# delldu/VSTNet

Measured on AMD Instinct MI355X. Metric: stylized frames/sec at 1024x1024 (1/2/4/8 GPU) + % HBM roofline, higher is better.
Workload: dtype bf16x3

## Files before the change

include/vstnet.h:

```cpp
#ifndef VSTNET_H
#define VSTNET_H

#include <stddef.h>
#include <stdint.h>

#ifdef __cplusplus
extern "C" {
#endif
#pragma GCC visibility push(default)

#define VST_OK 0
#define VST_E_ARG (-1)
#define VST_E_SHAPE (-2)
#define VST_E_MODE (-3)
#define VST_E_WORKSPACE (-4)

#define VST_PREC_BF16X3 0
#define VST_PREC_FP32 1
#define VST_PREC_F16X2 2

#define VST_PREC_F16X2H 3

#define VST_NUM_BLOCKS 32

// ... 160 lines not shown
int vst_cwct_factor_n_f64(const double* content_stats, const double* const* style_stats_host_array, const float* alphas_host,
                          int n_styles, float alpha_c, float eps, int N, double* affine, int* info, void* workspace,
                          size_t workspace_bytes, void* stream);
int vst_cwct_apply_n_f64(const float* x, float* y, int N, long L, const double* affine, const uint8_t* mask, int label,
                         void* stream);

#define VST_KERNEL_ID(cin, cout, stride) (((cin) << 16) | ((cout) << 4) | (stride))
#define VST_KERNEL_ALL (-1)
#define VST_KERNEL_PACK 1
#define VST_KERNEL_UNPACK 2
#define VST_KERNEL_SPREAD 3
#define VST_KERNEL_GATHER 4
#define VST_KERNEL_CWCT_STATS 5
#define VST_KERNEL_CWCT_FACTOR 6
#define VST_KERNEL_CWCT_APPLY 7
#define VST_KERNEL_PRESPLIT 8
int vst_profile_begin(int kernel_id, int max_records);
int vst_profile_end(double* total_ms, int* launches);
int vst_profile_end_table(int* ids, double* ms, int* launches, int cap, int* n_ids);

#define VST_OPT_STAGE3_LEAN 1
#define VST_OPT_STAGE3_PINGPONG 2
#define VST_OPT_STAGE3_WIDE 3
int vst_set_option(int option, int value);
int vst_get_option(int option);

#pragma GCC visibility pop
#ifdef __cplusplus
}
#endif
#endif
```

vstnet_amd/_lib.py:

```python
from __future__ import annotations

import ctypes as C
import glob
import os
import subprocess

PKG_DIR = os.path.dirname(os.path.abspath(__file__))
REPO_DIR = os.path.dirname(PKG_DIR)
LIB_PATH = os.environ.get("VSTNET_HIP_LIB") or os.path.join(PKG_DIR, "libvstnet_hip.so")
RESOURCES_PATH = os.path.join(PKG_DIR, "libvstnet_hip.resources.txt")
SOURCES = sorted(glob.glob(os.path.join(PKG_DIR, "csrc", "*.hip")))
HEADERS = sorted(glob.glob(os.path.join(PKG_DIR, "csrc", "*.h"))) + [os.path.join(REPO_DIR, "include", "vstnet.h")]

NUM_BLOCKS = 32
PREC_BF16X3 = 0
PREC_FP32 = 1
PREC_F16X2 = 2
PREC_F16X2H = 3

EXPORTS = [
    "vst_version", "vst_error_string", "vst_conv_packed_bytes", "vst_pack_conv", "vst_pack_input",
    "vst_unpack_output", "vst_pack_input_u8", "vst_unpack_output_u8", "vst_revnet_forward_u8", "vst_revnet_inverse_u8",
    "vst_spread", "vst_gather", "vst_block_tmp_bytes", "vst_block_apply",
    "vst_pass_workspace_bytes", "vst_revnet_forward", "vst_revnet_inverse",
# ... 4 lines not shown
    "vst_cwct_stats_code_workspace_bytes", "vst_cwct_stats_code", "vst_cwct_apply_code",
    "vst_mask_to_code", "vst_cwct_stats_labels_code_workspace_bytes", "vst_cwct_stats_labels_code", "vst_cwct_apply_labels_code",
    "vst_revnet_decode_labels", "vst_revnet_decode_labels_u8", "vst_pass_sub_batch",
    "vst_normalize_block", "vst_range_flags", "vst_range_flags_async",
    "vst_cwct_stats_f64_workspace_bytes", "vst_cwct_stats_f64", "vst_cwct_factor_f64_workspace_bytes", "vst_cwct_factor_f64",
    "vst_cwct_apply_f64",
    "vst_generic_conv", "vst_generic_squeeze", "vst_generic_unsqueeze", "vst_generic_copy_channels", "vst_generic_zero",
    "vst_set_option", "vst_get_option",
    "vst_cwct_stats_n_workspace_bytes", "vst_cwct_stats_n", "vst_cwct_factor_n_workspace_bytes", "vst_cwct_factor_n",
    "vst_cwct_prefactor_n", "vst_cwct_apply_n", "vst_cwct_stats_n_f64_workspace_bytes", "vst_cwct_stats_n_f64",
    "vst_cwct_factor_n_f64_workspace_bytes", "vst_cwct_factor_n_f64", "vst_cwct_apply_n_f64",
    "vst_max_frame_pixels", "vst_cwct_stats_code_rect", "vst_cwct_stats_labels_code_rect",
    "vst_colors_to_labels", "vst_label_hist", "vst_mask_prepare", "vst_remap_lut", "vst_apply_lut", "vst_label_plan_hist",
    "vst_cwct_factor_labels_keyed",
    "vst_label_plan_hists", "vst_cwct_factor_labels_mix", "vst_cwct_prefactor_labels",
]
MAX_STYLES = 8
MASK_OVERFLOW = 1
MASK_OUT_OF_TABLE = 2
LABEL_PLAN_BYTES = 2344
OPT_STAGE3_LEAN = 1
OPT_STAGE3_PINGPONG = 2
OPT_STAGE3_WIDE = 3
RANGE_SATURATED = 1
RANGE_WEIGHT = 2


PRECISIONS = {"bf16x3": PREC_BF16X3, "fp32": PREC_FP32, "f16x2": PREC_F16X2, "f16x2h": PREC_F16X2H}


def default_precision() -> str:
    p = os.environ.get("VST_PRECISION", "bf16x3")
    if p not in PRECISIONS:
        raise ValueError(f"VST_PRECISION must be one of {sorted(PRECISIONS)}")
    return p


class VstError(RuntimeError):
    pass


class ConvWeights(C.Structure):
    _fields_ = [("packed", C.c_void_p), ("bias", C.c_void_p)]


class BlockWeights(C.Structure):
# ... 205 lines not shown
```

vstnet_amd/csrc/conv.hip:

```cpp
#include <mutex>
#include <stdlib.h>
#include "common.h"

#ifndef VST_ABLATE
#define VST_ABLATE 0
#endif

struct ConvArgs {
    const float* in;
    float* out;
    const unsigned char* packed;
    const float* bias;
    int Hin, Win, Hout, Wout;
    int Wq;
    size_t in_img_stride;
    size_t out_img_stride;
    float sign;
    int tiles_x, tiles_y, tiles_total;
    const unsigned char* packed1;
    const float* bias1;
    unsigned char* out_sp;
    size_t out_sp_img_bytes;
    unsigned trace_base;
};

#ifndef VST_XCD_REMAP
#define VST_XCD_REMAP 1
#endif
#ifndef VST_PIPE_OLD_SPREAD
#define VST_PIPE_OLD_SPREAD 1
#endif
#ifndef VST_PIPE_NO_DEFER
#define VST_PIPE_NO_DEFER 0
#endif
#ifdef VST_TRACE
__device__ unsigned long long vst_trace_buf[4 * 16384];
__device__ unsigned long long* vst_trace_ptr;
__device__ unsigned vst_trace_cap;
static std::atomic<unsigned> vst_trace_host_n{0};
#define VST_TRACE_RESERVE(t_, grid_) (t_).trace_base = vst_trace_host_n.fetch_add((unsigned)(grid_));
#define VST_TRACE_BEGIN(which)                                                                                  \
    const unsigned long long trace_t0 = __builtin_amdgcn_s_memrealtime();
#define VST_TRACE_END_(which, cin_, cout_)                                                                      \
    if (VST_TRACE == (which) || VST_TRACE == 3) {                                                               \
        __builtin_amdgcn_s_waitcnt(0);                                                                          \
        asm volatile("s_waitcnt vmcnt(0)" ::: "memory");                                                       \
// ... 29 lines not shown
    (void)zero;
    vst_trace_host_n.store(0);
    return (int)e;
}
extern "C" __attribute__((visibility("default"))) int vst_trace_count(unsigned* n) { *n = vst_trace_host_n.load(); return 0; }
#else
#define VST_TRACE_BEGIN(which)
#define VST_TRACE_END(which)
#define VST_TRACE_END_(which, cin_, cout_)
#define VST_TRACE_RESERVE(t_, grid_)
#endif

__device__ __forceinline__ bool xcd_tile(const ConvArgs& a, int& bx, int& by, int& bz) {
    const int g = blockIdx.x, per = gridDim.x >> 3;
    const int n = VST_XCD_REMAP ? (g & 7) * per + (g >> 3) : g;
    if (n >= a.tiles_total) return false;
    bx = n % a.tiles_x;
    const int r = n / a.tiles_x;
    by = r % a.tiles_y;
    bz = r / a.tiles_y;
    return true;
}

template <int CIN, int COUT, int STRIDE, int MRO = 0>
struct ConvCfg {
    static constexpr int NT = COUT >= 64 ? 64 : 16;
    static constexpr int NB = NT / 16;
    static constexpr int COUTP = (COUT + 15) / 16 * 16;
    static constexpr int NCOT = COUTP / NT;
    static constexpr int MR = MRO ? MRO : (STRIDE == 2 ? 2 : 4);
    static constexpr int TH = 4 * MR, TW = 16;
    static constexpr int IH = (TH - 1) * STRIDE + 3, IW = (TW - 1) * STRIDE + 3;
    static constexpr int NSLOT = (IH * IW + 15) / 16 * 16;
    static constexpr int CC = CIN >= 32 ? 32 : CIN;
    static constexpr int NCHUNK = CIN / CC;
    static constexpr int CIG = CC >= 8 ? CC / 8 : 1;
#ifndef VST_ABLATE_KS16
#define VST_ABLATE_KS16 5
#endif
    static constexpr int KS = CIN >= 32 ? 9 : (CIN == 16 ? VST_ABLATE_KS16 : 2);
    static constexpr int A_PLANE = CIN == 4 ? NSLOT * 8 : CIG * NSLOT * 16;
    static constexpr int B_PLANE = KS * 4 * NT * 16;
    static constexpr int LDS_BYTES = 2 * A_PLANE + 2 * B_PLANE;
    static constexpr int LDS_BYTES_T2 = 2 * A_PLANE + B_PLANE;
    static_assert(LDS_BYTES <= 160 * 1024, "LDS budget");
};

__device__ __forceinline__ void split8_f16(const float4 v0, const float4 v1, uint4& hi, uint4& lo, float& amax) {
    const float f[8] = {v0.x, v0.y, v0.z, v0.w, v1.x, v1.y, v1.z, v1.w};
    u32x4 h, l;
    split8_sp(f, h, l, amax);
    hi = __builtin_bit_cast(uint4, h);
    lo = __builtin_bit_cast(uint4, l);
}

__device__ __forceinline__ void split4_f16(const float4 v, uint2& hi, uint2& lo, float& amax) {
    const float f[4] = {v.x, v.y, v.z, v.w};
    typedef __attribute__((ext_vector_type(4))) _Float16 f16x4;
    f16x4 h, l;
#ifndef VST_NO_RANGE_CHECK
    amax = fmaxf(fmaxf(amax, fabsf(f[0])), fmaxf(fmaxf(fabsf(f[1]), fabsf(f[2])), fabsf(f[3])));
#endif
#pragma unroll
// ... 77 lines not shown
            }
            *p = r;
        }
}

#define MFMA3(acc, wh, wl, xh, xl)                                              \
    acc = __builtin_amdgcn_mfma_f32_16x16x32_bf16(wh, xl, acc, 0, 0, 0);        \
    acc = __builtin_amdgcn_mfma_f32_16x16x32_bf16(wl, xh, acc, 0, 0, 0);        \
    acc = __builtin_amdgcn_mfma_f32_16x16x32_bf16(wh, xh, acc, 0, 0, 0)

#define MFMA_T(acc, wh, wl, xh, xl)                                                                                          \
    if constexpr (TERMS == 3) {                                                                                               \
        MFMA3(acc, wh, wl, xh, xl);                                                                                           \
    } else {                                                                                                                  \
        acc = __builtin_amdgcn_mfma_f32_16x16x32_f16(__builtin_bit_cast(f16x8, wh), __builtin_bit_cast(f16x8, xl), acc, 0, 0, 0); \
        acc = __builtin_amdgcn_mfma_f32_16x16x32_f16(__builtin_bit_cast(f16x8, wh), __builtin_bit_cast(f16x8, xh), acc, 0, 0, 0); \
    }
#define SPLIT8_T(v0_, v1_, h_, l_) { if constexpr (TERMS == 3) split8(v0_, v1_, h_, l_); else split8_f16(v0_, v1_, h_, l_, range_amax); }
#define SPLIT4_T(v_, h_, l_) { if constexpr (TERMS == 3) split4(v_, h_, l_); else split4_f16(v_, h_, l_, range_amax); }

#ifndef VST_EARLY_OLD
#define VST_EARLY_OLD 1
#endif
template <int CIN, int COUT, int STRIDE, bool IN_STATE, bool OUT_STATE, bool OUT_SP = false, int TERMS = 3, bool OUT_H16 = false>
__global__ __launch_bounds__(256) void conv_mfma_kernel(const ConvArgs a) {
    using C = ConvCfg<CIN, COUT, STRIDE>;
    extern __shared__ __attribute__((aligned(16))) unsigned char smem[];
    unsigned char* const a_hi = smem;
    unsigned char* const a_lo = smem + C::A_PLANE;
    unsigned char* const b_hi = smem + 2 * C::A_PLANE;
    unsigned char* const b_lo = TERMS == 3 ? b_hi + C::B_PLANE : b_hi;

    const int tid = threadIdx.x, lane = tid & 63, wave = tid >> 6;
    const int lrow = lane & 15, kg = lane >> 4;
    int bx, by, bz;
    if (!xcd_tile(a, bx, by, bz)) return;
    float range_amax = 0.f;
    VST_TRACE_BEGIN(2)
    const int tx0 = bx * C::TW, ty0 = by * C::TH;
    const int b = bz / C::NCOT, co0 = (bz % C::NCOT) * C::NT;

    const float* const in_img = a.in + (size_t)b * a.in_img_stride;
    const PackedConvLayout PL = packed_conv_layout(COUT, CIN);
    const unsigned char* const w_hi = a.packed + (TERMS == 3 ? PL.f32_bytes : PL.f16_offset);
    const unsigned char* const w_lo = w_hi + PL.frag_bytes;

    f32x4 acc[C::MR][C::NB];
#pragma unroll
    for (int m = 0; m < C::MR; ++m)
#pragma unroll
        for (int n = 0; n < C::NB; ++n) acc[m][n] = f32x4{0.f, 0.f, 0.f, 0.f};

    const int slot_base = (wave * C::MR * STRIDE) * C::IW + lrow * STRIDE;

    constexpr int A_ITEMS_T = CIN == 4 ? C::IH * C::IW : C::IH * C::IW * C::CIG;
    constexpr int AIT = (A_ITEMS_T + 255) / 256, NV = CIN == 4 ? 1 : 2;
    constexpr int W_ITEMS_T = C::KS * 4 * C::NT, WIT = (W_ITEMS_T + 255) / 256;
    typedef __attribute__((ext_vector_type(4))) unsigned u32x4;
    f32x4 areg[AIT][NV];
    u32x4 wreg[WIT][2];
#define F4(v_) make_float4((v_)[0], (v_)[1], (v_)[2], (v_)[3])
#define GEN_FETCH(chunk_)                                                                           \
    _Pragma("unroll") for (int it = 0; it < WIT; ++it) {                                           \
        int idx = it * 256 + tid;                                                                  \
        idx = idx < W_ITEMS_T ? idx : W_ITEMS_T - 1;                                               \
        const int co = idx % C::NT, r = idx / C::NT;                                               \
        const size_t src = ((size_t)((chunk_) * C::KS * 4 + r) * C::COUTP + co0 + co) * 16;        \
        wreg[it][0] = *(const u32x4*)(w_hi + src);                                                 \
        if (TERMS == 3) wreg[it][1] = *(const u32x4*)(w_lo + src);                                 \
    }                                                                                              \
    _Pragma("unroll") for (int it = 0; it < AIT; ++it) {                                           \
        int idx = it * 256 + tid;                                                                  \
        idx = idx < A_ITEMS_T ? idx : A_ITEMS_T - 1;                                               \
        const int cig = CIN == 4 ? 0 : idx % C::CIG, slot = CIN == 4 ? idx : idx / C::CIG;         \
        const int iy = slot / C::IW, ix = slot - iy * C::IW;                                       \
        const int gy = reflect_clamp(ty0 * STRIDE - 1 + iy, a.Hin);                                \
        const int gx = reflect_clamp(tx0 * STRIDE - 1 + ix, a.Win);                                \
        const size_t off = IN_STATE ? zc_offset(vst_level_of_channels(CIN), gy, gx, a.Wq)          \
                                    : ((size_t)gy * a.Win + gx) * CIN;                             \
        const float* p = in_img + off + (chunk_) * C::CC + cig * 8;                                \
        areg[it][0] = *(const f32x4*)p;                                                            \
        if (NV == 2) areg[it][NV - 1] = *(const f32x4*)(p + 4);                                    \
    }
#define GEN_LAND()                                                                                 \
    _Pragma("unroll") for (int it = 0; it < AIT; ++it) {                                           \
        int idx = it * 256 + tid;                                                                  \
        idx = idx < A_ITEMS_T ? idx : A_ITEMS_T - 1;                                               \
        if (CIN == 4) {                                                                            \
            uint2 h, l;                                                                            \
            SPLIT4_T(F4(areg[it][0]), h, l);                                                       \
            *(uint2*)(a_hi + idx * 8) = h;                                                         \
            *(uint2*)(a_lo + idx * 8) = l;                                                         \
// ... 3 lines not shown
            SPLIT8_T(F4(areg[it][0]), F4(areg[it][NV - 1]), h, l);                                 \
            *(uint4*)(a_hi + (cig * C::NSLOT + slot) * 16) = h;                                    \
            *(uint4*)(a_lo + (cig * C::NSLOT + slot) * 16) = l;                                    \
        }                                                                                          \
    }                                                                                              \
    _Pragma("unroll") for (int it = 0; it < WIT; ++it) {                                           \
        int idx = it * 256 + tid;                                                                  \
        idx = idx < W_ITEMS_T ? idx : W_ITEMS_T - 1;                                               \
        *(u32x4*)(b_hi + idx * 16) = wreg[it][0];                                                  \
        if (TERMS == 3) *(u32x4*)(b_lo + idx * 16) = wreg[it][1];                                  \
    }

    float* const out_img = a.out + (size_t)b * a.out_img_stride;
    float4 bias[C::NB], old[C::MR][C::NB];
    const bool interior = COUT % 16 == 0 && ty0 + C::TH <= a.Hout && tx0 + C::TW <= a.Wout;
    constexpr bool EARLY_OLD = OUT_STATE && VST_EARLY_OLD && C::MR * C::NB >= 16;
    auto fetch_old = [&]() __attribute__((always_inline)) {
        if (interior) load_old<COUT, C::MR, C::NB, true>(a, out_img, ty0 + wave * C::MR, tx0 + lrow, co0 + 4 * kg, old);
        else load_old<COUT, C::MR, C::NB>(a, out_img, ty0 + wave * C::MR, tx0 + lrow, co0 + 4 * kg, old);
    };

    GEN_FETCH(0);
    GEN_LAND();
#pragma unroll
    for (int chunk = 0; chunk < C::NCHUNK; ++chunk) {
        __syncthreads();
        if (chunk + 1 < C::NCHUNK) { GEN_FETCH(chunk + 1); }
        if (EARLY_OLD && chunk == C::NCHUNK - 1) fetch_old();

#pragma unroll
        for (int ks = 0; ks < C::KS; ++ks) {
            bf16x8 wh[C::NB], wl[C::NB];
#pragma unroll
            for (int n = 0; n < C::NB; ++n) {
                const int boff = ((ks * 4 + kg) * C::NT + n * 16 + lrow) * 16;
                wh[n] = __builtin_bit_cast(bf16x8, *(const uint4*)(b_hi + boff));
                if (TERMS == 3) wl[n] = __builtin_bit_cast(bf16x8, *(const uint4*)(b_lo + boff)); else wl[n] = wh[n];
            }
#pragma unroll
            for (int m = 0; m < C::MR; ++m) {
                bf16x8 xh, xl;
                if (CIN >= 32) {
                    const int dy = ks / 3, dx = ks - dy * 3;
                    const int slot = slot_base + (m * STRIDE + dy) * C::IW + dx;
                    const int aoff = (kg * C::NSLOT + slot) * 16;
                    xh = __builtin_bit_cast(bf16x8, *(const uint4*)(a_hi + aoff));
// ... 104 lines not shown
        xh = __builtin_bit_cast(bf16x8, make_uint4(h0.x, h0.y, h1.x, h1.y));
        if (!NO_LO) {
            const uint2 l0 = *(const uint2*)(img_lo + s0 * 8), l1 = *(const uint2*)(img_lo + s1 * 8);
            xl = __builtin_bit_cast(bf16x8, make_uint4(l0.x, l0.y, l1.x, l1.y));
        } else {
            xl = xh;
        }
    }
}

template <int MID, int CH, int TERMS = 3, int MR = 4, bool H16 = false>
struct PairCfg {
    using C7 = ConvCfg<MID, CH, 1, MR>;
    static constexpr int R1 = 20, N1SLOT = (4 * MR + 4) * R1, RW = 18, RH = 4 * MR + 2, NPX = RH * RW, NBLK = (NPX + 15) / 16;
    static constexpr int H1_PLANE = MID == 4 ? N1SLOT * 8 : C7::CIG * N1SLOT * 16;
    static constexpr int W4_PLANE = C7::KS * 4 * 16 * 16;
    static constexpr bool ALIAS = MID == 16;
    static constexpr int WPL = TERMS == 3 ? 2 : 1;
    static constexpr int H1W4 = (H16 ? 1 : 2) * H1_PLANE + WPL * W4_PLANE;
    static constexpr int U_BYTES = ALIAS ? (H1W4 > WPL * C7::B_PLANE ? H1W4 : WPL * C7::B_PLANE) : H1W4 + WPL * C7::B_PLANE;
    static constexpr int LDS_BYTES = 2 * C7::A_PLANE + U_BYTES;
};

template <int MID, int CH, int TERMS = 3, int MR = 4, bool H16 = false>
__global__ __launch_bounds__(256, (MID == 16 && TERMS == 2) ? 3 : 1) void conv_pair_kernel(const ConvArgs a) {
    static_assert(!H16 || TERMS == 2, "fp16 h1: the 2-term kernels only");
    using P = PairCfg<MID, CH, TERMS, MR, H16>;
    using C = typename P::C7;
    static_assert(C::NCHUNK == 1 && C::NCOT == 1, "single-chunk shapes");
    extern __shared__ __attribute__((aligned(16))) unsigned char smem[];
    unsigned char* const a_hi = smem;
    unsigned char* const a_lo = smem + C::A_PLANE;
    unsigned char* const u0 = smem + 2 * C::A_PLANE;
    unsigned char* const b_hi = P::ALIAS ? u0 : u0 + P::H1W4;
    unsigned char* const b_lo = TERMS == 3 ? b_hi + C::B_PLANE : b_hi;
    unsigned char* const h1_hi = u0;
    unsigned char* const h1_lo = H16 ? u0 : u0 + P::H1_PLANE;
    unsigned char* const w4s_hi = u0 + (H16 ? 1 : 2) * P::H1_PLANE;
    unsigned char* const w4s_lo = TERMS == 3 ? w4s_hi + P::W4_PLANE : w4s_hi;

    const int tid = threadIdx.x, lane = tid & 63, wave = tid >> 6;
    const int lrow = lane & 15, kg = lane >> 4;
    int bx, by, b;
    if (!xcd_tile(a, bx, by, b)) return;
    float range_amax = 0.f;
    VST_TRACE_BEGIN(1)
    const int tx0 = bx * C::TW, ty0 = by * C::TH;
    const int H = a.Hout, W = a.Wout;
    const float* const in_img = a.in + (size_t)b * a.in_img_stride;
// ... 26 lines not shown
        const int iy = slot / P::R1, ix = slot - iy * P::R1;
        const int gy = reflect_clamp(ty0 - 2 + iy, H), gx = reflect_clamp(tx0 - 2 + ix, W);
        if constexpr (H16) {
            const _Float16* p16 = (const _Float16*)a.in + (size_t)b * a.in_img_stride + ((size_t)gy * W + gx) * MID + cig * 8;
            if (MID == 4) { const uint2 v = *(const uint2*)p16; h16reg[it] = u32x4{v.x, v.y, 0u, 0u}; }
            else h16reg[it] = *(const u32x4*)p16;
        } else {
            const float* p = in_img + ((size_t)gy * W + gx) * MID + cig * 8;
            hreg[it][0] = *(const f32x4*)p;
            if (NV == 2) hreg[it][NV - 1] = *(const f32x4*)(p + 4);
        }
    }
#pragma unroll
    for (int it = 0; it < W7IT; ++it) {
        int idx = it * 256 + tid;
        idx = idx < W7_ITEMS ? idx : W7_ITEMS - 1;
        const int co = idx % C::NT, r = idx / C::NT;
        const size_t src = ((size_t)r * C::COUTP + co) * 16;
        w7reg[it][0] = *(const u32x4*)(w7_hi + src);
        if (TERMS == 3) w7reg[it][1] = *(const u32x4*)(w7_lo + src);
    }
    float4 bias[C::NB], old[C::MR][C::NB];
    const bool interior = ty0 + C::TH <= H && tx0 + C::TW <= W;
    constexpr bool EARLY_OLD = C::MR * C::NB >= 16 && TERMS == 3;
#define PAIR_FETCH_OLD()                                                                                         \
    if (interior) load_old<CH, C::MR, C::NB, true>(a, out_img, ty0 + wave * C::MR, tx0 + lrow, 4 * kg, old);   \
    else load_old<CH, C::MR, C::NB>(a, out_img, ty0 + wave * C::MR, tx0 + lrow, 4 * kg, old);
    if (EARLY_OLD) { PAIR_FETCH_OLD(); }

#define F4(v_) make_float4((v_)[0], (v_)[1], (v_)[2], (v_)[3])
#pragma unroll
    for (int it = 0; it < H1IT; ++it) {
        int idx = it * 256 + tid;
        idx = idx < H1_ITEMS ? idx : H1_ITEMS - 1;
        if constexpr (H16) {
            if (MID == 4) {
                *(uint2*)(h1_hi + idx * 8) = make_uint2(h16reg[it][0], h16reg[it][1]);
            } else {
                const int cig = idx % C::CIG, slot = idx / C::CIG;
                *(u32x4*)(h1_hi + (cig * P::N1SLOT + slot) * 16) = h16reg[it];
            }
        } else if (MID == 4) {
            uint2 h, l;
            SPLIT4_T(F4(hreg[it][0]), h, l);
            *(uint2*)(h1_hi + idx * 8) = h;
            *(uint2*)(h1_lo + idx * 8) = l;
        } else {
// ... 117 lines not shown
    for (int m = 0; m < C::MR; ++m)
#pragma unroll
        for (int n = 0; n < C::NB; ++n) acc[m][n] = f32x4{0.f, 0.f, 0.f, 0.f};
    const int slot_base = (wave * C::MR) * C::IW + lrow;
#pragma unroll
    for (int ks = 0; ks < C::KS; ++ks) {
        bf16x8 wh[C::NB], wl[C::NB];
#pragma unroll
        for (int n = 0; n < C::NB; ++n) {
            const int boff = ((ks * 4 + kg) * C::NT + n * 16 + lrow) * 16;
            wh[n] = __builtin_bit_cast(bf16x8, *(const uint4*)(b_hi + boff));
            wl[n] = __builtin_bit_cast(bf16x8, *(const uint4*)(b_lo + boff));
        }
#pragma unroll
        for (int m = 0; m < C::MR; ++m) {
            bf16x8 xh, xl;
            read_x_small<MID>(a_hi, a_lo, C::NSLOT, slot_base + m * C::IW, C::IW, ks, kg, xh, xl);
#pragma unroll
            for (int n = 0; n < C::NB; ++n) { MFMA_T(acc[m][n], wh[n], wl[n], xh, xl); }
        }
    }
    load_bias<CH, C::NB>(a, 4 * kg, bias);
    if constexpr (TERMS == 2) vst_note_range(range_amax);
    if (!EARLY_OLD) { PAIR_FETCH_OLD(); }
#undef PAIR_FETCH_OLD
    if (interior) store_tile<CH, true, C::MR, C::NB, true>(a, out_img, ty0 + wave * C::MR, tx0 + lrow, 4 * kg, acc, bias, old);
    else store_tile<CH, true, C::MR, C::NB>(a, out_img, ty0 + wave * C::MR, tx0 + lrow, 4 * kg, acc, bias, old);
    VST_TRACE_END_(1, MID, CH)
}

#ifdef VST_PP_STAMP
__device__ unsigned long long vst_pp_stamps[2 * 32 * 8];
extern "C" __attribute__((visibility("default"))) int vst_pp_stamps_dump(unsigned long long* host) {
    return (int)hipMemcpyFromSymbol(host, HIP_SYMBOL(vst_pp_stamps), sizeof(vst_pp_stamps));
}
#define PP_STAMP(grp_, st_, k_)                                                                                  \
    if (blockIdx.x == 128 && lane == 0 && (wave & 3) == 0 && (st_) < 32) {                                       \
        asm volatile("s_waitcnt lgkmcnt(0)" ::: "memory");                                                      \
        vst_pp_stamps[((grp_) * 32 + (st_)) * 8 + (k_)] = __builtin_amdgcn_s_memtime();                          \
    }
__device__ unsigned long long vst_pp_clk[4];
extern "C" __attribute__((visibility("default"))) int vst_pp_clk_dump(unsigned long long* host) {
    return (int)hipMemcpyFromSymbol(host, HIP_SYMBOL(vst_pp_clk), sizeof(vst_pp_clk));
}
#define PP_CLK(i_)                                                                                               \
    if (blockIdx.x == 128 && threadIdx.x == 0) {                                                                 \
// ... 665 lines not shown
    (void)hipEventRecord(g_prof_ev[2 * rec], st);
    return rec;
}

void vst_prof_close(int rec, hipStream_t st) {
    std::lock_guard<std::mutex> lk(g_prof_mu);
    if (rec < g_prof_count) (void)hipEventRecord(g_prof_ev[2 * rec + 1], st);
}

#ifndef VST_LEAN_DEFAULT
#define VST_LEAN_DEFAULT 0
#endif
static std::atomic<int> g_opt_lean{[] { const char* e = getenv("VST_LEAN"); return e && (e[0] == '0' || e[0] == '1') ? e[0] - '0' : VST_LEAN_DEFAULT; }()};
static bool vst_lean_stage3() { return g_opt_lean.load(std::memory_order_relaxed) != 0; }
#ifndef VST_WIDE_DEFAULT
#define VST_WIDE_DEFAULT 1
#endif
static std::atomic<int> g_opt_wide{[] { const char* e = getenv("VST_WIDE"); return e && (e[0] == '0' || e[0] == '1') ? e[0] - '0' : VST_WIDE_DEFAULT; }()};
#ifndef VST_PINGPONG_DEFAULT
#define VST_PINGPONG_DEFAULT 0
#endif
static std::atomic<int> g_opt_pp{[] { const char* e = getenv("VST_PINGPONG"); return e && (e[0] == '0' || e[0] == '1') ? e[0] - '0' : VST_PINGPONG_DEFAULT; }()};

template <int CIN, int COUT, int STRIDE, bool IN_STATE, bool OUT_STATE>
static int launch_conv(const ConvArgs& a, int B, int precision, hipStream_t st, bool out_h16 = false) {
    if (precision == VST_PREC_FP32) {
        const size_t total = (size_t)B * a.Hout * a.Wout * COUT;
        size_t blocks = (total + 255) / 256;
        if (blocks > 65536) blocks = 65536;
        conv_fp32_kernel<IN_STATE, OUT_STATE><<<dim3((unsigned)blocks), 256, 0, st>>>(a, CIN, COUT, STRIDE, B);
        VST_RETURN_IF_LAUNCH_FAILED();
        return VST_OK;
    }
    if (precision != VST_PREC_BF16X3 && !vst_is_f16(precision)) return VST_E_MODE;
    vst_prof_scope prof(VST_KERNEL_ID(CIN, COUT, STRIDE), st);
    if constexpr (CIN >= 64 && COUT >= 64 && STRIDE == 1) {
        ConvArgs t = a;
        t.tiles_x = (a.Wout + 15) / 16;
        if (vst_lean_stage3()) {
            using C = PipeCfg<CIN, COUT, 4>;
            auto kern = conv_pipe_kernel<CIN, COUT, IN_STATE, OUT_STATE, 4>;
            static std::atomic<unsigned> attr_done{0};
            if (int rc_ = vst_ensure_dynamic_lds((const void*)kern, (int)(C::LDS_BYTES), &attr_done)) return rc_;
            t.tiles_y = (a.Hout + C::TH - 1) / C::TH; t.tiles_total = t.tiles_x * t.tiles_y * B;
            VST_TRACE_RESERVE(t, (t.tiles_total + 7) / 8 * 8)
            kern<<<dim3((t.tiles_total + 7) / 8 * 8), C::NTHR, C::LDS_BYTES, st>>>(t);
// ... 14 lines not shown
            if (int rc_ = vst_ensure_dynamic_lds((const void*)kern, lds, &attr_done)) return rc_;
            t.tiles_y = (a.Hout + C::TH - 1) / C::TH; t.tiles_total = t.tiles_x * t.tiles_y * B;
            VST_TRACE_RESERVE(t, (t.tiles_total + 7) / 8 * 8)
            kern<<<dim3((t.tiles_total + 7) / 8 * 8), C::NTHR, lds, st>>>(t);
#endif
        } else {
            using C = PipeCfg<CIN, COUT>;
            auto kern = conv_pipe_kernel<CIN, COUT, IN_STATE, OUT_STATE>;
            static std::atomic<unsigned> attr_done{0};
            if (int rc_ = vst_ensure_dynamic_lds((const void*)kern, (int)(C::LDS_BYTES), &attr_done)) return rc_;
            t.tiles_y = (a.Hout + C::TH - 1) / C::TH; t.tiles_total = t.tiles_x * t.tiles_y * B;
            VST_TRACE_RESERVE(t, (t.tiles_total + 7) / 8 * 8)
            kern<<<dim3((t.tiles_total + 7) / 8 * 8), C::NTHR, C::LDS_BYTES, st>>>(t);
        }
    } else {
        using C = ConvCfg<CIN, COUT, STRIDE>;
        constexpr bool T2_SHAPE = (CIN == 64 && COUT == 16) || (CIN == 16 && COUT == 16 && STRIDE == 2) || (CIN == 16 && COUT == 4);
        const bool t2 = T2_SHAPE && vst_is_f16(precision);
        constexpr bool H16_SHAPE = T2_SHAPE && !OUT_STATE;
        const bool h16 = t2 && out_h16 && H16_SHAPE;
        auto kern = h16 ? conv_mfma_kernel<CIN, COUT, STRIDE, IN_STATE, OUT_STATE, false, T2_SHAPE ? 2 : 3, H16_SHAPE>
                  : t2 ? conv_mfma_kernel<CIN, COUT, STRIDE, IN_STATE, OUT_STATE, false, T2_SHAPE ? 2 : 3>
                       : conv_mfma_kernel<CIN, COUT, STRIDE, IN_STATE, OUT_STATE, false, 3>;
        const int lds = t2 ? C::LDS_BYTES_T2 : C::LDS_BYTES;
        static std::atomic<unsigned> attr_done[3];
        if (int rc_ = vst_ensure_dynamic_lds((const void*)kern, lds, &attr_done[h16 ? 2 : (t2 ? 1 : 0)])) return rc_;
        ConvArgs t = a;
        t.tiles_x = (a.Wout + C::TW - 1) / C::TW; t.tiles_y = (a.Hout + C::TH - 1) / C::TH;
        t.tiles_total = t.tiles_x * t.tiles_y * B * C::NCOT;
        VST_TRACE_RESERVE(t, (t.tiles_total + 7) / 8 * 8)
        kern<<<dim3((t.tiles_total + 7) / 8 * 8), 256, lds, st>>>(t);
    }
    VST_RETURN_IF_LAUNCH_FAILED();
    return VST_OK;
}

static int launch_conv_s2_planes(const ConvArgs& a, int B, hipStream_t st) {
    using C = ConvCfg<64, 64, 2>;
    vst_prof_scope prof(VST_KERNEL_ID(64, 64, 2), st);
    auto kern = conv_mfma_kernel<64, 64, 2, true, false, true, 2>;
    static std::atomic<unsigned> attr_done{0};
    if (int rc_ = vst_ensure_dynamic_lds((const void*)kern, (int)(C::LDS_BYTES_T2), &attr_done)) return rc_;
    ConvArgs t = a;
    t.tiles_x = (a.Wout + C::TW - 1) / C::TW; t.tiles_y = (a.Hout + C::TH - 1) / C::TH;
    t.tiles_total = t.tiles_x * t.tiles_y * B * C::NCOT;
    VST_TRACE_RESERVE(t, (t.tiles_total + 7) / 8 * 8)
    kern<<<dim3((t.tiles_total + 7) / 8 * 8), 256, C::LDS_BYTES_T2, st>>>(t);
    VST_RETURN_IF_LAUNCH_FAILED();
    return VST_OK;
}

#ifndef VST_PAIR
#define VST_PAIR 1
#endif
#ifndef VST_PAIR_MR2_T3
#define VST_PAIR_MR2_T3 0
#endif
#ifndef VST_PAIR_MR2
#define VST_PAIR_MR2 0
#endif
template <int MID, int CH>
static int launch_pair(const ConvArgs& a, int B, int precision, hipStream_t st) {
    constexpr int T2 = 2;
    const bool t2 = T2 == 2 && vst_is_f16(precision);
    if (precision == VST_PREC_F16X2H) {
        using P = PairCfg<MID, CH, 2, 4, true>;
        vst_prof_scope prof(VST_KERNEL_ID(MID, CH, 1), st);
        auto kern = conv_pair_kernel<MID, CH, 2, 4, true>;
        static std::atomic<unsigned> attr_h16{0};
        if (int rc_ = vst_ensure_dynamic_lds((const void*)kern, P::LDS_BYTES, &attr_h16)) return rc_;
        ConvArgs t = a;
        t.tiles_x = (a.Wout + 15) / 16; t.tiles_y = (a.Hout + 15) / 16; t.tiles_total = t.tiles_x * t.tiles_y * B;
        VST_TRACE_RESERVE(t, (t.tiles_total + 7) / 8 * 8)
        kern<<<dim3((t.tiles_total + 7) / 8 * 8), 256, P::LDS_BYTES, st>>>(t);
        VST_RETURN_IF_LAUNCH_FAILED();
        return VST_OK;
    }
    vst_prof_scope prof(VST_KERNEL_ID(MID, CH, 1), st);
    constexpr int MRT = (MID == 16 && VST_PAIR_MR2) ? 2 : 4;
    constexpr int MRT3 = (MID == 16 && VST_PAIR_MR2_T3) ? 2 : 4;
    auto kern = t2 ? conv_pair_kernel<MID, CH, T2, MRT> : conv_pair_kernel<MID, CH, 3, MRT3>;
    const int lds = t2 ? PairCfg<MID, CH, T2, MRT>::LDS_BYTES : PairCfg<MID, CH, 3, MRT3>::LDS_BYTES;
    const int th = t2 ? 4 * MRT : 4 * MRT3;
    static std::atomic<unsigned> attr_done[2];
    if (int rc_ = vst_ensure_dynamic_lds((const void*)kern, lds, &attr_done[t2 ? 1 : 0])) return rc_;
    ConvArgs t = a;
    t.tiles_x = (a.Wout + 15) / 16; t.tiles_y = (a.Hout + th - 1) / th; t.tiles_total = t.tiles_x * t.tiles_y * B;
    VST_TRACE_RESERVE(t, (t.tiles_total + 7) / 8 * 8)
    kern<<<dim3((t.tiles_total + 7) / 8 * 8), 256, lds, st>>>(t);
    VST_RETURN_IF_LAUNCH_FAILED();
    return VST_OK;
}

template <int CH, int STRIDE>
static int run_block(const vst_block_weights* w, int direction, int precision, float* dst, const float* src,
                     float* tmp, int B, int H, int W, hipStream_t st) {
    constexpr int LV = CH == 16 ? 0 : (CH == 64 ? 1 : 2);
    constexpr int MID = CH / 4;
    constexpr int IN_CH = STRIDE == 1 ? CH : CH / 4;
    const int Ho = H >> LV, Wo = W >> LV;
    const size_t state_img = (size_t)H * W * 16;
    const size_t mid_img = (size_t)Ho * Wo * MID;
    float* h1 = tmp;
    float* h2 = tmp + (size_t)B * mid_img;
    ConvArgs a{};
    a.Wq = W >> 2;
    a.in = src; a.out = h1; a.packed = (const unsigned char*)w->conv[0].packed; a.bias = w->conv[0].bias;
    a.Hin = Ho * STRIDE; a.Win = Wo * STRIDE; a.Hout = Ho; a.Wout = Wo;
    a.in_img_stride = state_img; a.out_img_stride = mid_img; a.sign = 0.f;
    if constexpr (CH == 256 && STRIDE == 2) {
        if (vst_is_f16(precision)) {
            const size_t mid_bytes = (size_t)Ho * Wo * 64 * 4, state_bytes = (size_t)Ho * Wo * 256 * 4;
            unsigned char* const h1p = (unsigned char*)tmp;
            unsigned char* const h2p = h1p + (size_t)B * mid_bytes;
            unsigned char* const planes_a = h2p + (size_t)B * mid_bytes;
            (void)state_bytes;
            a.out_sp = h1p; a.out_sp_img_bytes = mid_bytes;
            int rc2 = launch_conv_s2_planes(a, B, st);
            if (rc2) return rc2;
            const int h2_single = precision == VST_PREC_F16X2H;
            rc2 = vst3_conv_mid(&w->conv[1], h1p, h2p, h2_single, B, H, W, st);
            if (rc2) return rc2;
            return vst3_conv_out(&w->conv[2], h2p, h2_single, dst, direction > 0 ? planes_a : nullptr, direction > 0 ? 1.f : -1.f,
                                 B, H, W, st);
        }
    }
    const bool h16 = CH <= 64 && VST_PAIR && precision == VST_PREC_F16X2H;
    int rc = launch_conv<IN_CH, MID, STRIDE, true, false>(a, B, precision, st, h16);
    if (rc) return rc;
    if constexpr (CH <= 64 && VST_PAIR) {
        if (precision != VST_PREC_FP32) {
            a.in = h1; a.out = dst; a.Hin = Ho; a.Win = Wo; a.in_img_stride = mid_img; a.out_img_stride = state_img;
            a.packed = (const unsigned char*)w->conv[2].packed; a.bias = w->conv[2].bias;
            a.packed1 = (const unsigned char*)w->conv[1].packed; a.bias1 = w->conv[1].bias;
            a.sign = direction > 0 ? 1.f : -1.f;
            return launch_pair<MID, CH>(a, B, precision, st);
        }
    }
    a.in = h1; a.out = h2; a.packed = (const unsigned char*)w->conv[1].packed; a.bias = w->conv[1].bias;
    a.Hin = Ho; a.Win = Wo; a.in_img_stride = mid_img;
    rc = launch_conv<MID, MID, 1, false, false>(a, B, precision, st);
    if (rc) return rc;
    a.in = h2; a.out = dst; a.packed = (const unsigned char*)w->conv[2].packed; a.bias = w->conv[2].bias;
    a.out_img_stride = state_img; a.sign = direction > 0 ? 1.f : -1.f;
    return launch_conv<MID, CH, 1, false, true>(a, B, precision, st);
}

static const int kBlockChannel[VST_NUM_BLOCKS] = {16, 16, 16, 16, 16, 16, 16, 16, 16, 16, 64, 64, 64, 64, 64, 64,
                                                  64, 64, 64, 64, 256, 256, 256, 256, 256, 256, 256, 256, 256, 256,
                                                  256, 256};
static const int kBlockStride[VST_NUM_BLOCKS] = {1, 1, 1, 1, 1, 1, 1, 1, 1, 1, 2, 1, 1, 1, 1, 1,
                                                 1, 1, 1, 1, 2, 1, 1, 1, 1, 1, 1, 1, 1, 1, 1, 1};

VST_DEFINE_TU_RANGE(vst_range_tu_conv)

extern "C" {

int vst_set_option(int option, int value) {
    if (option == VST_OPT_STAGE3_LEAN) g_opt_lean.store(value != 0, std::memory_order_relaxed);
    else if (option == VST_OPT_STAGE3_WIDE) g_opt_wide.store(value != 0, std::memory_order_relaxed);
    else if (option == VST_OPT_STAGE3_PINGPONG && VST_WITH_PINGPONG) g_opt_pp.store(value != 0, std::memory_order_relaxed);
    else return VST_E_ARG;
    return VST_OK;
}

int vst_get_option(int option) {
    if (option == VST_OPT_STAGE3_LEAN) return g_opt_lean.load(std::memory_order_relaxed);
    if (option == VST_OPT_STAGE3_WIDE) return g_opt_wide.load(std::memory_order_relaxed);
    if (option == VST_OPT_STAGE3_PINGPONG && VST_WITH_PINGPONG) return g_opt_pp.load(std::memory_order_relaxed);
    return VST_E_ARG;
}

int vst_range_flags(unsigned* flags_host, int reset) {
    if (!flags_host) return VST_E_ARG;
    hipError_t e = hipDeviceSynchronize();
    if (e != hipSuccess) return (int)e;
    unsigned v = 0;
    if (int rc = vst_range_tu_conv(&v, reset)) return rc;
    if (int rc = vst_range_tu_conv3(&v, reset)) return rc;
    if (int rc = vst_range_tu_layout(&v, reset)) return rc;
    if (int rc = vst_range_tu_cwct(&v, reset)) return rc;
    *flags_host = v;
    return VST_OK;
}

int vst_range_flags_async(unsigned* flags4_dev, void* stream) {
    if (!flags4_dev) return VST_E_ARG;
    hipStream_t st = (hipStream_t)stream;
    if (int rc = vst_range_tu_conv_async(flags4_dev + 0, st)) return rc;
    if (int rc = vst_range_tu_conv3_async(flags4_dev + 1, st)) return rc;
    if (int rc = vst_range_tu_layout_async(flags4_dev + 2, st)) return rc;
    return vst_range_tu_cwct_async(flags4_dev + 3, st);
// ... 108 lines not shown
        else
            rc = vst_block_apply(&w->blocks[k], kBlockChannel[k], kBlockStride[k], +1, precision, s[k & 1], s[1 - (k & 1)],
                                 tmp, B, H, W, stream);
        if (rc) return rc;
    }
    return VST_OK;
}

static int revnet_forward_chunk(const vst_net_weights* w, const float* x, const uint8_t* x_u8, float* z, void* workspace,
                                int B, int C_in, int H, int W, int sp_steps, int precision, void* stream) {
    float* s[2];
    s[0] = (float*)workspace;
    s[1] = s[0] + (size_t)B * H * W * 16;
    float* tmp = s[1] + (size_t)B * H * W * 16;
    const int rc = forward_blocks(w, x, x_u8, s, tmp, B, C_in, H, W, precision, stream);
    if (rc) return rc;
    return vst_spread(s[0], s[1], z, B, H, W, sp_steps, stream);
}

static int inverse_blocks(const vst_net_weights* w, float* x, uint8_t* x_u8, float* const s[2], float* tmp, int B, int C_out,
                          int H, int W, int precision, void* stream) {
    const bool sp = vst_is_f16(precision);
    int rc = VST_OK;
    for (int k = VST_NUM_BLOCKS - 1; k >= 0; --k) {
        if (sp && k >= 21)
            rc = vst3_block256(&w->blocks[k], -1, precision, s[k & 1], s[1 - (k & 1)], tmp, VST_NUM_BLOCKS - 1 - k, 1, B, H, W,
                               stream);
        else
            rc = vst_block_apply(&w->blocks[k], kBlockChannel[k], kBlockStride[k], -1, precision, s[k & 1], s[1 - (k & 1)],
                                 tmp, B, H, W, stream);
        if (rc) return rc;
    }
    return x_u8 ? vst_unpack_output_u8(s[0], x_u8, B, H, W, stream) : vst_unpack_output(s[0], x, B, C_out, H, W, stream);
}

static int revnet_inverse_chunk(const vst_net_weights* w, const float* z, float* x, uint8_t* x_u8, void* workspace, int B,
                                int C_out, int H, int W, int sp_steps, int precision, void* stream) {
    float* s[2];
    s[0] = (float*)workspace;
    s[1] = s[0] + (size_t)B * H * W * 16;
    float* tmp = s[1] + (size_t)B * H * W * 16;
    const bool sp = vst_is_f16(precision);
    const int rc = sp ? vst3_gather_planes(z, vst3_plane_buffer(tmp, 0, B, H, W), s[1], B, H, W, sp_steps, stream)
                      : vst_gather(z, s[0], s[1], B, H, W, sp_steps, stream);
    if (rc) return rc;
    return inverse_blocks(w, x, x_u8, s, tmp, B, C_out, H, W, precision, stream);
}

static int revnet_encode_any(const vst_net_weights* w, const float* x, const uint8_t* x_u8, float* code, void* workspace, int B,
                             int C_in, int H, int W, int precision, void* stream) {
// ... 187 lines not shown
```

Before: 217.5.

## Fold 3x3 taps for 16-to-4 conv and fuse final block with RGB output

Adds a tap-folded form of the 16-channel-in, 4-channel-out conv. It treats the spatial taps as MFMA output rows and sums the shifted partial results through LDS, so the MFMA does not waste lanes padding 4 output channels to 16. It also fuses the last inverse block's pair kernel with the output unpack, writing planar float or u8 RGB directly and skipping the separate unpack pass and the state write. Both paths are on by default and controlled by new options. The cost is extra LDS transposes and syncs in the folded kernel and more special-case code paths.

```diff
diff --git a/include/vstnet.h b/include/vstnet.h
--- a/include/vstnet.h
+++ b/include/vstnet.h
@@ -206,6 +206,8 @@
 #define VST_OPT_STAGE3_LEAN 1
 #define VST_OPT_STAGE3_PINGPONG 2
 #define VST_OPT_STAGE3_WIDE 3
+#define VST_OPT_STAGE1_FOLD 4
+#define VST_OPT_OUT_RGB 5
 int vst_set_option(int option, int value);
 int vst_get_option(int option);
 
diff --git a/vstnet_amd/_lib.py b/vstnet_amd/_lib.py
--- a/vstnet_amd/_lib.py
+++ b/vstnet_amd/_lib.py
@@ -50,6 +50,8 @@
 OPT_STAGE3_LEAN = 1
 OPT_STAGE3_PINGPONG = 2
 OPT_STAGE3_WIDE = 3
+OPT_STAGE1_FOLD = 4
+OPT_OUT_RGB = 5
 RANGE_SATURATED = 1
 RANGE_WEIGHT = 2
 
diff --git a/vstnet_amd/csrc/conv.hip b/vstnet_amd/csrc/conv.hip
--- a/vstnet_amd/csrc/conv.hip
+++ b/vstnet_amd/csrc/conv.hip
@@ -22,6 +22,9 @@
     unsigned char* out_sp;
     size_t out_sp_img_bytes;
     unsigned trace_base;
+    float* rgb;
+    unsigned char* rgb_u8;
+    int rgb_c;
 };
 
 #ifndef VST_XCD_REMAP
@@ -97,7 +100,7 @@
     return true;
 }
 
-template <int CIN, int COUT, int STRIDE, int MRO = 0>
+template <int CIN, int COUT, int STRIDE, int MRO = 0, int KSO = 0>
 struct ConvCfg {
     static constexpr int NT = COUT >= 64 ? 64 : 16;
     static constexpr int NB = NT / 16;
@@ -113,7 +116,7 @@
 #ifndef VST_ABLATE_KS16
 #define VST_ABLATE_KS16 5
 #endif
-    static constexpr int KS = CIN >= 32 ? 9 : (CIN == 16 ? VST_ABLATE_KS16 : 2);
+    static constexpr int KS = KSO ? KSO : (CIN >= 32 ? 9 : (CIN == 16 ? VST_ABLATE_KS16 : 2));
     static constexpr int A_PLANE = CIN == 4 ? NSLOT * 8 : CIG * NSLOT * 16;
     static constexpr int B_PLANE = KS * 4 * NT * 16;
     static constexpr int LDS_BYTES = 2 * A_PLANE + 2 * B_PLANE;
@@ -237,9 +240,12 @@
 #ifndef VST_EARLY_OLD
 #define VST_EARLY_OLD 1
 #endif
-template <int CIN, int COUT, int STRIDE, bool IN_STATE, bool OUT_STATE, bool OUT_SP = false, int TERMS = 3, bool OUT_H16 = false>
+template <int CIN, int COUT, int STRIDE, bool IN_STATE, bool OUT_STATE, bool OUT_SP = false, int TERMS = 3, bool OUT_H16 = false,
+          bool FOLD = false>
 __global__ __launch_bounds__(256) void conv_mfma_kernel(const ConvArgs a) {
-    using C = ConvCfg<CIN, COUT, STRIDE>;
+    static_assert(!FOLD || (CIN == 16 && COUT == 4 && STRIDE == 1 && TERMS == 3 && !OUT_STATE && !OUT_SP && !OUT_H16),
+                  "tap-folded form: conv.1 of the 16-channel blocks, bf16x3");
+    using C = ConvCfg<CIN, COUT, STRIDE, 0, FOLD ? 2 : 0>;
     extern __shared__ __attribute__((aligned(16))) unsigned char smem[];
     unsigned char* const a_hi = smem;
     unsigned char* const a_lo = smem + C::A_PLANE;
@@ -280,9 +286,19 @@
         int idx = it * 256 + tid;                                                                  \
         idx = idx < W_ITEMS_T ? idx : W_ITEMS_T - 1;                                               \
         const int co = idx % C::NT, r = idx / C::NT;                                               \
-        const size_t src = ((size_t)((chunk_) * C::KS * 4 + r) * C::COUTP + co0 + co) * 16;        \
-        wreg[it][0] = *(const u32x4*)(w_hi + src);                                                 \
-        if (TERMS == 3) wreg[it][1] = *(const u32x4*)(w_lo + src);                                 \
+        if constexpr (FOLD) {                                                                      \
+            const int ty = 2 * (r >> 2) + ((r >> 1) & 1), tx = co >> 2;           \
+            const bool live = ty < 3 && tx < 3;                                                    \
+            const int tap = live ? 3 * ty + tx : 0;                                                \
+            const size_t src = ((size_t)((tap >> 1) * 4 + (tap & 1) * 2 + (r & 1)) * 16 + (co & 3)) * 16; \
+            const u32x4 h_ = *(const u32x4*)(w_hi + src), l_ = *(const u32x4*)(w_lo + src);        \
+            wreg[it][0] = live ? h_ : u32x4{0u, 0u, 0u, 0u};                                       \
+            wreg[it][1] = live ? l_ : u32x4{0u, 0u, 0u, 0u};                                       \
+        } else {                                                                                   \
+            const size_t src = ((size_t)((chunk_) * C::KS * 4 + r) * C::COUTP + co0 + co) * 16;    \
+            wreg[it][0] = *(const u32x4*)(w_hi + src);                                             \
+            if (TERMS == 3) wreg[it][1] = *(const u32x4*)(w_lo + src);                             \
+        }                                                                                          \
     }                                                                                              \
     _Pragma("unroll") for (int it = 0; it < AIT; ++it) {                                           \
         int idx = it * 256 + tid;                                                                  \
@@ -332,6 +348,53 @@
 
     GEN_FETCH(0);
     GEN_LAND();
+    if constexpr (FOLD) {
+        constexpr int NPX = C::MR * C::IW, NBLK = (NPX + 15) / 16;
+        static_assert(4 * NBLK * 16 * 12 * 4 <= 2 * C::A_PLANE, "the transposed accumulators fit the image region");
+        __syncthreads();
+        f32x4 facc[NBLK];
+#pragma unroll
+        for (int j = 0; j < NBLK; ++j) facc[j] = f32x4{0.f, 0.f, 0.f, 0.f};
+#pragma unroll
+        for (int ks = 0; ks < C::KS; ++ks) {
+            const int boff = ((ks * 4 + kg) * 16 + lrow) * 16;
+            const bf16x8 wh = __builtin_bit_cast(bf16x8, *(const uint4*)(b_hi + boff));
+            const bf16x8 wl = __builtin_bit_cast(bf16x8, *(const uint4*)(b_lo + boff));
+            int ty = 2 * ks + (kg >> 1);
+            ty = ty > 2 ? 2 : ty;
+#pragma unroll
+            for (int j = 0; j < NBLK; ++j) {
+                int q = j * 16 + lrow;
+                q = q < NPX ? q : NPX - 1;
+                const int aoff = ((kg & 1) * C::NSLOT + (wave * C::MR + ty) * C::IW + q) * 16;
+                const bf16x8 xh = __builtin_bit_cast(bf16x8, *(const uint4*)(a_hi + aoff));
+                const bf16x8 xl = __builtin_bit_cast(bf16x8, *(const uint4*)(a_lo + aoff));
+                MFMA3(facc[j], wh, wl, xh, xl);
+            }
+        }
+        __syncthreads();
+        float* const sc = (float*)smem + wave * (NBLK * 16 * 12);
+        if (kg < 3) {
+#pragma unroll
+            for (int j = 0; j < NBLK; ++j) *(f32x4*)(sc + ((j * 16 + lrow) * 3 + kg) * 4) = facc[j];
+        }
+        __syncthreads();
+        const int q0 = kg * C::IW + lrow;
+        const f32x4 d0 = *(const f32x4*)(sc + ((q0 + 0) * 3 + 0) * 4);
+        const f32x4 d1 = *(const f32x4*)(sc + ((q0 + 1) * 3 + 1) * 4);
+        const f32x4 d2 = *(const f32x4*)(sc + ((q0 + 2) * 3 + 2) * 4);
+        const float4 bs = *(const float4*)a.bias;
+        const int oy = ty0 + wave * C::MR + kg, ox = tx0 + lrow;
+        if (oy < a.Hout && ox < a.Wout) {
+            float4 r = make_float4((d0[0] + d1[0]) + d2[0] + bs.x, (d0[1] + d1[1]) + d2[1] + bs.y,
+                                   (d0[2] + d1[2]) + d2[2] + bs.z, (d0[3] + d1[3]) + d2[3] + bs.w);
+            r.x = r.x > 0.f ? r.x : 0.f; r.y = r.y > 0.f ? r.y : 0.f;
+            r.z = r.z > 0.f ? r.z : 0.f; r.w = r.w > 0.f ? r.w : 0.f;
+            *(float4*)(a.out + (size_t)b * a.out_img_stride + ((size_t)oy * a.Wout + ox) * COUT) = r;
+        }
+        VST_TRACE_END_(2, CIN, COUT)
+        return;
+    }
 #pragma unroll
     for (int chunk = 0; chunk < C::NCHUNK; ++chunk) {
         __syncthreads();
@@ -482,9 +545,10 @@
     static constexpr int LDS_BYTES = 2 * C7::A_PLANE + U_BYTES;
 };
 
-template <int MID, int CH, int TERMS = 3, int MR = 4, bool H16 = false>
+template <int MID, int CH, int TERMS = 3, int MR = 4, bool H16 = false, bool OUT_RGB = false>
 __global__ __launch_bounds__(256, (MID == 16 && TERMS == 2) ? 3 : 1) void conv_pair_kernel(const ConvArgs a) {
     static_assert(!H16 || TERMS == 2, "fp16 h1: the 2-term kernels only");
+    static_assert(!OUT_RGB || (MID == 4 && CH == 16), "image output: the 16-channel blocks only");
     using P = PairCfg<MID, CH, TERMS, MR, H16>;
     using C = typename P::C7;
     static_assert(C::NCHUNK == 1 && C::NCOT == 1, "single-chunk shapes");
@@ -557,7 +621,7 @@
     }
     float4 bias[C::NB], old[C::MR][C::NB];
     const bool interior = ty0 + C::TH <= H && tx0 + C::TW <= W;
-    constexpr bool EARLY_OLD = C::MR * C::NB >= 16 && TERMS == 3;
+    constexpr bool EARLY_OLD = C::MR * C::NB >= 16 && TERMS == 3 && !OUT_RGB;
 #define PAIR_FETCH_OLD()                                                                                         \
     if (interior) load_old<CH, C::MR, C::NB, true>(a, out_img, ty0 + wave * C::MR, tx0 + lrow, 4 * kg, old);   \
     else load_old<CH, C::MR, C::NB>(a, out_img, ty0 + wave * C::MR, tx0 + lrow, 4 * kg, old);
@@ -721,6 +785,36 @@
     }
     load_bias<CH, C::NB>(a, 4 * kg, bias);
     if constexpr (TERMS == 2) vst_note_range(range_amax);
+    if constexpr (OUT_RGB) {
+        const int ox = tx0 + lrow, nc = a.rgb_u8 ? 3 : a.rgb_c;
+        const size_t plane = (size_t)H * W;
+#pragma unroll
+        for (int m = 0; m < C::MR; ++m) {
+            const int oy = ty0 + wave * C::MR + m;
+            if (oy >= H || ox >= W || 4 * kg >= nc) continue;
+            const float4 o = *(const float4*)(out_img + zc_offset(0, oy, ox, a.Wq) + 4 * kg);
+            float4 r = make_float4(acc[m][0][0] + bias[0].x, acc[m][0][1] + bias[0].y, acc[m][0][2] + bias[0].z,
+                                   acc[m][0][3] + bias[0].w);
+            r = make_float4(o.x + a.sign * r.x, o.y + a.sign * r.y, o.z + a.sign * r.z, o.w + a.sign * r.w);
+            const float c[4] = {r.x, r.y, r.z, r.w};
+            if (a.rgb_u8) {
+                unsigned char* dst = a.rgb_u8 + ((size_t)b * plane + (size_t)oy * W + ox) * 3;
+#pragma unroll
+                for (int k = 0; k < 3; ++k) {
+                    float t = c[k] * 255.f;
+                    t = t < 0.f ? 0.f : (t > 255.f ? 255.f : t);
+                    dst[k] = (unsigned char)t;
+                }
+            } else {
+                float* dst = a.rgb + ((size_t)b * a.rgb_c + 4 * kg) * plane + (size_t)oy * W + ox;
+#pragma unroll
+                for (int k = 0; k < 4; ++k)
+                    if (4 * kg + k < nc) dst[k * plane] = c[k];
+            }
+        }
+        VST_TRACE_END_(1, MID, CH)
+        return;
+    }
     if (!EARLY_OLD) { PAIR_FETCH_OLD(); }
 #undef PAIR_FETCH_OLD
     if (interior) store_tile<CH, true, C::MR, C::NB, true>(a, out_img, ty0 + wave * C::MR, tx0 + lrow, 4 * kg, acc, bias, old);
@@ -1432,6 +1526,15 @@
 #endif
 static std::atomic<int> g_opt_pp{[] { const char* e = getenv("VST_PINGPONG"); return e && (e[0] == '0' || e[0] == '1') ? e[0] - '0' : VST_PINGPONG_DEFAULT; }()};
 
+#ifndef VST_FOLD16_DEFAULT
+#define VST_FOLD16_DEFAULT 1
+#endif
+static std::atomic<int> g_opt_fold{[] { const char* e = getenv("VST_FOLD16"); return e && (e[0] == '0' || e[0] == '1') ? e[0] - '0' : VST_FOLD16_DEFAULT; }()};
+#ifndef VST_OUT_RGB_DEFAULT
+#define VST_OUT_RGB_DEFAULT 1
+#endif
+static std::atomic<int> g_opt_rgb{[] { const char* e = getenv("VST_OUT_RGB"); return e && (e[0] == '0' || e[0] == '1') ? e[0] - '0' : VST_OUT_RGB_DEFAULT; }()};
+
 template <int CIN, int COUT, int STRIDE, bool IN_STATE, bool OUT_STATE>
 static int launch_conv(const ConvArgs& a, int B, int precision, hipStream_t st, bool out_h16 = false) {
     if (precision == VST_PREC_FP32) {
@@ -1492,9 +1595,18 @@
         auto kern = h16 ? conv_mfma_kernel<CIN, COUT, STRIDE, IN_STATE, OUT_STATE, false, T2_SHAPE ? 2 : 3, H16_SHAPE>
                   : t2 ? conv_mfma_kernel<CIN, COUT, STRIDE, IN_STATE, OUT_STATE, false, T2_SHAPE ? 2 : 3>
                        : conv_mfma_kernel<CIN, COUT, STRIDE, IN_STATE, OUT_STATE, false, 3>;
-        const int lds = t2 ? C::LDS_BYTES_T2 : C::LDS_BYTES;
-        static std::atomic<unsigned> attr_done[3];
-        if (int rc_ = vst_ensure_dynamic_lds((const void*)kern, lds, &attr_done[h16 ? 2 : (t2 ? 1 : 0)])) return rc_;
+        int lds = t2 ? C::LDS_BYTES_T2 : C::LDS_BYTES;
+        constexpr bool FOLD_SHAPE = CIN == 16 && COUT == 4 && STRIDE == 1 && !OUT_STATE;
+        bool fold = false;
+        if constexpr (FOLD_SHAPE) {
+            if (!t2 && g_opt_fold.load(std::memory_order_relaxed)) {
+                fold = true;
+                kern = conv_mfma_kernel<CIN, COUT, STRIDE, IN_STATE, OUT_STATE, false, 3, false, true>;
+                lds = ConvCfg<CIN, COUT, STRIDE, 0, 2>::LDS_BYTES;
+            }
+        }
+        static std::atomic<unsigned> attr_done[4];
+        if (int rc_ = vst_ensure_dynamic_lds((const void*)kern, lds, &attr_done[fold ? 3 : (h16 ? 2 : (t2 ? 1 : 0))])) return rc_;
         ConvArgs t = a;
         t.tiles_x = (a.Wout + C::TW - 1) / C::TW; t.tiles_y = (a.Hout + C::TH - 1) / C::TH;
         t.tiles_total = t.tiles_x * t.tiles_y * B * C::NCOT;
@@ -1533,6 +1645,24 @@
 static int launch_pair(const ConvArgs& a, int B, int precision, hipStream_t st) {
     constexpr int T2 = 2;
     const bool t2 = T2 == 2 && vst_is_f16(precision);
+    if constexpr (MID == 4) {
+        if (a.rgb || a.rgb_u8) {
+            using P = PairCfg<MID, CH, 3>;
+            static_assert(P::LDS_BYTES >= PairCfg<MID, CH, 2>::LDS_BYTES && P::LDS_BYTES >= PairCfg<MID, CH, 2, 4, true>::LDS_BYTES, "");
+            vst_prof_scope prof(VST_KERNEL_ID(MID, CH, 1), st);
+            const int form = precision == VST_PREC_F16X2H ? 2 : (t2 ? 1 : 0);
+            auto kern = form == 2 ? conv_pair_kernel<MID, CH, 2, 4, true, true>
+                      : form == 1 ? conv_pair_kernel<MID, CH, 2, 4, false, true> : conv_pair_kernel<MID, CH, 3, 4, false, true>;
+            static std::atomic<unsigned> attr_rgb[3];
+            if (int rc_ = vst_ensure_dynamic_lds((const void*)kern, P::LDS_BYTES, &attr_rgb[form])) return rc_;
+            ConvArgs t = a;
+            t.tiles_x = (a.Wout + 15) / 16; t.tiles_y = (a.Hout + 15) / 16; t.tiles_total = t.tiles_x * t.tiles_y * B;
+            VST_TRACE_RESERVE(t, (t.tiles_total + 7) / 8 * 8)
+            kern<<<dim3((t.tiles_total + 7) / 8 * 8), 256, P::LDS_BYTES, st>>>(t);
+            VST_RETURN_IF_LAUNCH_FAILED();
+            return VST_OK;
+        }
+    }
     if (precision == VST_PREC_F16X2H) {
         using P = PairCfg<MID, CH, 2, 4, true>;
         vst_prof_scope prof(VST_KERNEL_ID(MID, CH, 1), st);
@@ -1564,7 +1694,8 @@
 
 template <int CH, int STRIDE>
 static int run_block(const vst_block_weights* w, int direction, int precision, float* dst, const float* src,
-                     float* tmp, int B, int H, int W, hipStream_t st) {
+                     float* tmp, int B, int H, int W, hipStream_t st, float* rgb = nullptr, uint8_t* rgb_u8 = nullptr,
+                     int rgb_c = 0) {
     constexpr int LV = CH == 16 ? 0 : (CH == 64 ? 1 : 2);
     constexpr int MID = CH / 4;
     constexpr int IN_CH = STRIDE == 1 ? CH : CH / 4;
@@ -1604,6 +1735,7 @@
             a.packed = (const unsigned char*)w->conv[2].packed; a.bias = w->conv[2].bias;
             a.packed1 = (const unsigned char*)w->conv[1].packed; a.bias1 = w->conv[1].bias;
             a.sign = direction > 0 ? 1.f : -1.f;
+            a.rgb = rgb; a.rgb_u8 = rgb_u8; a.rgb_c = rgb_c;
             return launch_pair<MID, CH>(a, B, precision, st);
         }
     }
@@ -1630,6 +1762,8 @@
     if (option == VST_OPT_STAGE3_LEAN) g_opt_lean.store(value != 0, std::memory_order_relaxed);
     else if (option == VST_OPT_STAGE3_WIDE) g_opt_wide.store(value != 0, std::memory_order_relaxed);
     else if (option == VST_OPT_STAGE3_PINGPONG && VST_WITH_PINGPONG) g_opt_pp.store(value != 0, std::memory_order_relaxed);
+    else if (option == VST_OPT_STAGE1_FOLD) g_opt_fold.store(value != 0, std::memory_order_relaxed);
+    else if (option == VST_OPT_OUT_RGB) g_opt_rgb.store(value != 0, std::memory_order_relaxed);
     else return VST_E_ARG;
     return VST_OK;
 }
@@ -1638,6 +1772,8 @@
     if (option == VST_OPT_STAGE3_LEAN) return g_opt_lean.load(std::memory_order_relaxed);
     if (option == VST_OPT_STAGE3_WIDE) return g_opt_wide.load(std::memory_order_relaxed);
     if (option == VST_OPT_STAGE3_PINGPONG && VST_WITH_PINGPONG) return g_opt_pp.load(std::memory_order_relaxed);
+    if (option == VST_OPT_STAGE1_FOLD) return g_opt_fold.load(std::memory_order_relaxed);
+    if (option == VST_OPT_OUT_RGB) return g_opt_rgb.load(std::memory_order_relaxed);
     return VST_E_ARG;
 }
 
@@ -1792,10 +1928,19 @@
                           int H, int W, int precision, void* stream) {
     const bool sp = vst_is_f16(precision);
     int rc = VST_OK;
+    const bool rgb0 = precision != VST_PREC_FP32 && VST_PAIR && g_opt_rgb.load(std::memory_order_relaxed) != 0;
+    if (rgb0) {
+        if ((!x && !x_u8) || !vst_shape_ok(B, H, W) || (!x_u8 && (C_out < 1 || C_out > 16))) return VST_E_ARG;
+        for (int i = 0; i < 3; ++i)
+            if (!w->blocks[0].conv[i].packed || !w->blocks[0].conv[i].bias) return VST_E_ARG;
+    }
     for (int k = VST_NUM_BLOCKS - 1; k >= 0; --k) {
         if (sp && k >= 21)
             rc = vst3_block256(&w->blocks[k], -1, precision, s[k & 1], s[1 - (k & 1)], tmp, VST_NUM_BLOCKS - 1 - k, 1, B, H, W,
                                stream);
+        else if (k == 0 && rgb0)
+            return run_block<16, 1>(&w->blocks[0], -1, precision, s[0], s[1], tmp, B, H, W, (hipStream_t)stream,
+                                    x_u8 ? nullptr : x, x_u8, C_out);
         else
             rc = vst_block_apply(&w->blocks[k], kBlockChannel[k], kBlockStride[k], -1, precision, s[k & 1], s[1 - (k & 1)],
                                  tmp, B, H, W, stream);
```

New measurement: 221.0 (median of 6 runs). 1.02x the previous value.
